# courtois-neuromod/phantom_vlb

Measured on AMD Instinct MI355X. Metric: clips/sec fine-tune VideoLLaMA2-7B+LoRA->2k-voxel head, 1/2/4/8 MI355X, higher is better.
Workload: dtype bf16; 1 GPU; configs[2]: VideoLLaMA2-7B + LoRA r=16 + 2k-voxel head, bf16; clips_per_gpu=3, global_batch=3, seq_len=2048, frames=12, num_target=2048, weights=random-init, comm=none

## Files before the change

include/vlb.h:

```cpp
#ifndef VLB_H
#define VLB_H

#include <stdint.h>

#ifdef __cplusplus
extern "C" {
#endif
#if defined(__GNUC__) || defined(__clang__)
#pragma GCC visibility push(default)
#endif

#define VLB_OK 0
#define VLB_ERR_INVALID (-1)
#define VLB_ERR_LAUNCH (-2)

#define VLB_ABI_VERSION 2

#define VLB_ACT_NONE 0
#define VLB_ACT_QUICK_GELU 1
#define VLB_ACT_GELU 2
#define VLB_ACT_SILU 3
#define VLB_ACT_SWIGLU_PAIR 4
#define VLB_ACT_SWIGLU_BWD 5

int vlb_abi_version(void);
const char* vlb_last_error(void);

int vlb_gemm_bf16(const void* A, int lda, const void* W, int ldw, void* C, int ldc, int M, int N, int K,
                  const void* bias, const void* residual, int ldr, int act, const void* A2, int lda2,
                  const void* W2, int ldw2, int K2, void* stream);

int vlb_gemm_bf16_ws(const void* A, int lda, const void* W, int ldw, void* C, int ldc, int M, int N, int K,
                     const void* bias, const void* residual, int ldr, int act, const void* A2, int lda2,
                     const void* W2, int ldw2, int K2, void* ws, int64_t ws_bytes, void* stream);
int vlb_gemm_swiglu_save(const void* A, int lda, const void* W_il, int ldw, void* H, int ldh, void* GU, int ldgu, int M, int N,
                         int K, const void* A2, int lda2, const void* W2_il, int ldw2, int K2, void* ws, int64_t ws_bytes,
                         void* stream);
int64_t vlb_gemm_workspace_bytes(void);
int vlb_gemm_plan(int M, int N, int K, int K2, int with_workspace);

int vlb_gemm_bf16_masked_pair(const void* A, int lda, const void* W, int ldw, void* C, int ldc, int M, int N, int K,
                              const void* A2, int lda2, const void* W2, int ldw2, float drop_p, uint32_t seed,
                              void* stream);

int vlb_gemm_bf16_masked_pair_ws(const void* A, int lda, const void* W, int ldw, void* C, int ldc, int M, int N, int K,
                                 const void* A2, int lda2, const void* W2, int ldw2, float drop_p, uint32_t seed,
                                 void* ws, int64_t ws_bytes, void* stream);

int vlb_gemm_masked_pair_swiglu_bwd(const void* dY, int lddy, const void* Wt, int ldw, const void* gu, int ldgu, void* dgu,
                                    int lddgu, int M, int ff, int K, const void* U, int ldu, const void* At, int ldat,
                                    float drop_p, uint32_t seed, void* ws, int64_t ws_bytes, void* stream);

int vlb_gemm_kernel_choice(int M, int N, int K, int K2);

int vlb_transpose_bf16(const void* in, void* out, int R, int C, void* stream);

int vlb_attention_fwd(const void* q, int ldq, const void* k, int ldk, const void* v, int ldv, void* out, int ldo,
                      float* lse, const uint8_t* key_mask, int B, int S, int Hq, int Hkv, int D, int causal,
                      float scale, const int* cu_rows, void* stream);

int vlb_attention_bwd(const void* q, int ldq, const void* k, int ldk, const void* v, int ldv, const void* out,
                      int ldo, const void* dout, int lddo, const float* lse, const uint8_t* key_mask, void* dq,
                      int lddq, void* dk, int lddk, void* dv, int lddv, float* delta, float* dq_acc, int B, int S,
                      int Hq, int Hkv, int D, int causal, float scale, const int* cu_rows, int total_rows,
                      void* stream);

int vlb_rmsnorm_fwd(const void* x, const void* w, void* y, int rows, int dim, float eps, void* stream);
int vlb_rmsnorm_bwd(const void* x, const void* w, const void* dy, const void* dx_in, void* dx, int rows, int dim,
                    float eps, void* stream);
int vlb_layernorm_fwd(const void* x, const void* w, const void* b, const void* residual, void* y, int rows, int dim,
                      float eps, int act, void* stream);

int vlb_rope_inplace(void* x, int ld, const float* cos_t, const float* sin_t, int rows, int S, int heads, int D,
                     int sign, const int* pos, void* stream);
int vlb_swiglu_fwd(const void* gu, void* out, int rows, int ff, void* stream);
int vlb_swiglu_bwd(const void* gu, const void* dout, void* dgu, int rows, int ff, void* stream);
int vlb_add_bf16(const void* a, const void* b, void* y, int64_t n, void* stream);

int vlb_patchify(const float* vision, void* patches, int N, int H, int W, int P, int Kpad, void* stream);
int vlb_vit_assemble(const void* patch_emb, const void* cls, const void* pos, void* tokens, int N, int G, int D,
                     void* stream);
int vlb_drop_cls(const void* tokens, void* out, int N, int G, int D, void* stream);

int vlb_dwconv3x3(const void* x, const void* w, void* y, int N, int H, int W, int C, void* stream);
int vlb_se_pool(const void* x, void* pooled, int N, int HW, int C, void* stream);
int vlb_se_scale(const void* x, const void* gate, void* y, int N, int HW, int C, void* stream);
int vlb_im2col3d_k2s2p1(const void* x, void* cols, int B, int T, int H, int W, int C, void* stream);

int vlb_splice_embed(const int64_t* ids, const void* embed_w, const void* video_tokens, void* embeds,
                     uint8_t* key_mask, int* err_flag, int B, int L, int Nv, int D, int64_t video_id, int vocab,
                     const int* cu_rows, int* row_pos, void* stream);
int vlb_weight_mask(const int64_t* padvals, const double* vis_w, const double* lang_w, float* wmask, int B, int F,
                    int Lw, int tokens_per_frame, int S, int round_bf16, void* stream);

int vlb_head_partial_rows(int S);
int64_t vlb_head_ws_floats(int B, int S, int E, int V);
int vlb_head_fwd(const void* hidden, const float* wmask, const void* ln1_w, const void* ln1_b, const void* ln2_w,
                 const void* ln2_b, const void* ridge_w, const void* ridge_b, const float* y, const float* keep_scale,
                 float* ws, float* stats, float* pooled_raw, float* sumw, float* zhat, float* ln2_rstd, void* z,
                 float* pred, float* loss_terms, int B, int S, int E, int V, float eps, float l2_lambda, const int* cu_rows,
                 void* stream);
int vlb_head_bwd(const void* hidden, const float* wmask, const void* ln1_w, const void* ln2_w, const void* ridge_w,
                 const float* y, const float* keep_scale, const float* stats, const float* pooled_raw,
                 const float* sumw, const float* zhat, const float* ln2_rstd, const void* z, const float* pred,
                 float* d_ridge_w, float* d_ridge_b, float* d_ln2_w, float* d_ln2_b, float* d_ln1_w, float* d_ln1_b,
                 float* ws, float* dz_ws, float* dpooled_ws, void* dhidden, int B, int S, int E, int V, float eps,
                 float l2_lambda, float loss_scale, float l2_scale, const int* cu_rows, int total_rows, void* stream);

int vlb_feature_cache_store(const float* pooled_raw, const float* sumw, const int32_t* rows, float* cache_pooled,
                            float* cache_sumw, int B, int E, int n_rows, void* stream);
int vlb_head_fwd_cached(const float* cache_pooled, const float* cache_sumw, const int32_t* rows, const void* ln1_w,
                        const void* ln1_b, const void* ln2_w, const void* ln2_b, const void* ridge_w, const void* ridge_b,
                        const float* y, const float* keep_scale, float* ws, float* pooled_raw, float* sumw, float* zhat,
                        float* ln2_rstd, void* z, float* pred, float* loss_terms, int B, int E, int V, int n_rows, float eps,
                        float l2_lambda, void* stream);
int vlb_head_bwd_cached(const void* ln1_w, const void* ln2_w, const void* ridge_w, const float* y, const float* keep_scale,
                        const float* pooled_raw, const float* sumw, const float* zhat, const float* ln2_rstd, const void* z,
                        const float* pred, float* d_ridge_w, float* d_ridge_b, float* d_ln2_w, float* d_ln2_b, float* d_ln1_w,
                        float* d_ln1_b, float* ws, float* dz_ws, float* dpooled_ws, int B, int E, int V, float eps,
                        float l2_lambda, float loss_scale, float l2_scale, void* stream);

#define VLB_LOSS_MSE 0
#define VLB_LOSS_COSINE 1
#define VLB_LOSS_PEARSON 2
int vlb_head_loss_fwd(const float* pred, const float* y, const float* ws, float* rowstat, float* loss_terms, float* loss_aux,
                      int B, int S, int E, int V, int loss_kind, float l2_lambda, void* stream);
int vlb_head_bwd_loss(const void* hidden, const float* wmask, const void* ln1_w, const void* ln2_w, const void* ridge_w,
                      const float* y, const float* keep_scale, const float* stats, const float* pooled_raw,
                      const float* sumw, const float* zhat, const float* ln2_rstd, const void* z, const float* pred,
                      float* d_ridge_w, float* d_ridge_b, float* d_ln2_w, float* d_ln2_b, float* d_ln1_w, float* d_ln1_b,
                      float* ws, float* dz_ws, float* dpooled_ws, void* dhidden, int B, int S, int E, int V, float eps,
                      float l2_lambda, float loss_scale, float l2_scale, const int* cu_rows, int total_rows, void* stream,
                      int loss_kind, const float* rowstat);
int vlb_head_bwd_cached_loss(const void* ln1_w, const void* ln2_w, const void* ridge_w, const float* y, const float* keep_scale,
                             const float* pooled_raw, const float* sumw, const float* zhat, const float* ln2_rstd,
                             const void* z, const float* pred, float* d_ridge_w, float* d_ridge_b, float* d_ln2_w,
                             float* d_ln2_b, float* d_ln1_w, float* d_ln1_b, float* ws, float* dz_ws, float* dpooled_ws, int B,
                             int E, int V, float eps, float l2_lambda, float loss_scale, float l2_scale, void* stream,
                             int loss_kind, const float* rowstat);

int vlb_head_pool(const void* hidden, const float* wmask, float* ws, float* stats, float* pooled_raw, float* sumw, int B,
                  int S, int E, float eps, const int* cu_rows, void* stream);
int vlb_feature_cache_gather(const float* cache_pooled, const float* cache_sumw, const int32_t* rows, float* pooled_raw,
                             float* sumw, int B, int E, int n_rows, void* stream);
int vlb_head_mix_fwd(const float* p_stack, const void* a, float* alpha, float* pooled_raw, int K, int B, int E,
                     void* stream);
int64_t vlb_head_mix_ws_floats(int K, int B, int E);
int vlb_head_mix_bwd(const float* p_stack, const float* draw, const float* alpha, float* d_a, float* draw_stack, float* ws,
                     int K, int B, int E, void* stream);
int vlb_head_dhidden(const void* hidden, const float* wmask, const float* stats, const float* draw, void* dx, int B, int S,
                     int E, const int* cu_rows, int total_rows, int accumulate, void* stream);

int vlb_lora_down(const void* x, int ldx, const void* A, void* t, int ldt, int M, int K, int R, float scale,
                  float drop_p, const uint32_t* seeds_host, void* stream);
int vlb_lora_merge(const void* W, int ldw, void* Wm, int ldwm, const void* Bt, const void* A, int N, int K, int R, float scale,
                   int row_map, void* stream);
int vlb_lora_dx_masked(const void* u, int ldu, const void* At, int ldat, void* dx, int lddx, int M, int K, int R, float drop_p,
                       const uint32_t* seeds_host, void* stream);
int64_t vlb_wgrad_u_ws_floats(int M, int K);
int vlb_wgrad_skinny_u(const void* G, int ldg, const void* X, int ldx, float* dW, float* ws, int M, int K, float alpha,
                       float beta, const void* Bt, float u_scale, void* u, int ldu, float* u_ws, void* stream);
int vlb_wgrad_skinny_u_multi(const void* G, int ldg, const void* X, int ldx, int M, int nproj, const int* cols, float* const* dW,
                             const void* const* Bt, float* ws, float alpha, float beta, float u_scale, void* u, int ldu,
                             float* u_ws, void* stream);
int vlb_transpose16_scatter(const void* jobs, int n_jobs, void* stream);
int vlb_wgrad_splits(int M);
int vlb_wgrad_skinny(const void* G, int ldg, const void* X, int ldx, float* dW, float* ws, int M, int N, int K,
                     float alpha, float beta, float drop_p, const uint32_t* seeds_host, void* stream);

// ... 77 lines not shown
```

phantom_vlb_amd/_lib.py:

```python
from __future__ import annotations

import ctypes
import os
from ctypes import c_char_p, c_double, c_float, c_int, c_int64, c_void_p

import torch

_HERE = os.path.dirname(os.path.abspath(__file__))
LIB_PATH = os.environ.get("VLB_LIB") or os.path.join(_HERE, "libvlb.so")
IS_PRODUCT_LIB = os.path.abspath(LIB_PATH) == os.path.join(_HERE, "libvlb.so")

P, I, F, L = c_void_p, c_int, c_float, c_int64

SIGNATURES = {
    "vlb_abi_version": [],
    "vlb_last_error": [],
    "vlb_gemm_bf16": [P, I, P, I, P, I, I, I, I, P, P, I, I, P, I, P, I, I, P],
    "vlb_gemm_bf16_ws": [P, I, P, I, P, I, I, I, I, P, P, I, I, P, I, P, I, I, P, L, P],
    "vlb_gemm_swiglu_save": [P, I, P, I, P, I, P, I, I, I, I, P, I, P, I, I, P, L, P],
    "vlb_gemm_workspace_bytes": [],
    "vlb_gemm_plan": [I, I, I, I, I],
    "vlb_gemm_kernel_choice": [I, I, I, I],
    "vlb_transpose_bf16": [P, P, I, I, P],
    "vlb_attention_fwd": [P, I, P, I, P, I, P, I, P, P, I, I, I, I, I, I, F, P, P],
    "vlb_attention_bwd": [P, I, P, I, P, I, P, I, P, I, P, P, P, I, P, I, P, I, P, P, I, I, I, I, I, I, F, P, I, P],
    "vlb_rmsnorm_fwd": [P, P, P, I, I, F, P],
    "vlb_rmsnorm_bwd": [P, P, P, P, P, I, I, F, P],
    "vlb_layernorm_fwd": [P, P, P, P, P, I, I, F, I, P],
    "vlb_rope_inplace": [P, I, P, P, I, I, I, I, I, P, P],
    "vlb_swiglu_fwd": [P, P, I, I, P],
    "vlb_swiglu_bwd": [P, P, P, I, I, P],
    "vlb_add_bf16": [P, P, P, L, P],
    "vlb_patchify": [P, P, I, I, I, I, I, P],
    "vlb_vit_assemble": [P, P, P, P, I, I, I, P],
    "vlb_drop_cls": [P, P, I, I, I, P],
    "vlb_dwconv3x3": [P, P, P, I, I, I, I, P],
    "vlb_se_pool": [P, P, I, I, I, P],
    "vlb_se_scale": [P, P, P, I, I, I, P],
    "vlb_im2col3d_k2s2p1": [P, P, I, I, I, I, I, P],
    "vlb_splice_embed": [P, P, P, P, P, P, I, I, I, I, L, I, P, P, P],
    "vlb_weight_mask": [P, P, P, P, I, I, I, I, I, I, P],
    "vlb_head_partial_rows": [I],
    "vlb_head_ws_floats": [I, I, I, I],
    "vlb_head_fwd": [P] * 19 + [I, I, I, I, F, F, P, P],
    "vlb_head_bwd": [P] * 24 + [I, I, I, I, F, F, F, F, P, I, P],
    "vlb_feature_cache_store": [P] * 5 + [I, I, I, P],
    "vlb_head_fwd_cached": [P] * 19 + [I, I, I, I, F, F, P],
    "vlb_head_bwd_cached": [P] * 20 + [I, I, I, F, F, F, F, P],
    "vlb_head_loss_fwd": [P] * 6 + [I, I, I, I, I, F, P],
    "vlb_head_bwd_loss": [P] * 24 + [I, I, I, I, F, F, F, F, P, I, P, I, P],
    "vlb_head_bwd_cached_loss": [P] * 20 + [I, I, I, F, F, F, F, P, I, P],
    "vlb_head_pool": [P] * 6 + [I, I, I, F, P, P],
    "vlb_feature_cache_gather": [P] * 5 + [I, I, I, P],
    "vlb_head_mix_fwd": [P] * 4 + [I, I, I, P],
    "vlb_head_mix_ws_floats": [I, I, I],
    "vlb_head_mix_bwd": [P] * 6 + [I, I, I, P],
    "vlb_head_dhidden": [P] * 5 + [I, I, I, P, I, I, P],
    "vlb_gemm_bf16_masked_pair": [P, I, P, I, P, I, I, I, I, P, I, P, I, F, ctypes.c_uint32, P],
    "vlb_gemm_masked_pair_swiglu_bwd": [P, I, P, I, P, I, P, I, I, I, I, P, I, P, I, F, ctypes.c_uint32, P, L, P],
    "vlb_gemm_bf16_masked_pair_ws": [P, I, P, I, P, I, I, I, I, P, I, P, I, F, ctypes.c_uint32, P, L, P],
    "vlb_wgrad_u_ws_floats": [I, I],
    "vlb_wgrad_skinny_u": [P, I, P, I, P, P, I, I, F, F, P, F, P, I, P, P],
    "vlb_wgrad_skinny_u_multi": [P, I, P, I, I, I, P, P, P, P, F, F, F, P, I, P, P],
    "vlb_transpose16_scatter": [P, I, P],
    "vlb_wgrad_splits": [I],
    "vlb_wgrad_skinny": [P, I, P, I, P, P, I, I, I, F, F, F, P, P],
    "vlb_lora_down": [P, I, P, P, I, I, I, I, F, F, P, P],
    "vlb_lora_merge": [P, I, P, I, P, P, I, I, I, F, I, P],
    "vlb_lora_dx_masked": [P, I, P, I, P, I, I, I, I, F, P, P],
    "vlb_sumsq_ws_floats": [],
    "vlb_grad_sumsq": [P, L, P, P, P],
    "vlb_adamw_step": [P, P, P, P, P, L, F, F, F, F, F, I, P, F, P],
    "vlb_grad_accum": [P, P, L, I, P, P, P],
    "vlb_grad_accum_bf16": [P, P, L, I, P, P, P],
    "vlb_dropout_keep_scale": [P, L, F, ctypes.c_uint32, P],
    "vlb_transpose_pad": [P, I, P, I, I, I, I, P],
    "vlb_norm_bwd_ws_floats": [I, I],
    "vlb_colsum_ws_floats": [I, I],
    "vlb_rmsnorm_bwd_dw": [P, P, P, P, I, I, F, P],
    "vlb_rmsnorm_bwd_full_ws_floats": [I, I],
    "vlb_rmsnorm_bwd_full": [P, P, P, P, P, P, P, I, I, F, P],
    "vlb_layernorm_bwd": [P, P, P, P, P, P, P, P, P, P, I, I, F, I, P],
    "vlb_act_fwd": [P, P, L, I, P],
    "vlb_act_bwd": [P, P, P, L, I, P],
    "vlb_colsum": [P, I, P, P, I, I, P],
    "vlb_embed_grad": [P, I, P, P, P, I, P, I, P],
    "vlb_grad_sumsq_bf16": [P, L, P, P, P],
    "vlb_adamw_step_g16": [P, P, P, P, P, L, F, F, F, F, F, I, P, F, P],
    "vlb_dwconv3x3_bwd_w_ws_floats": [I, I, I],
    "vlb_dwconv3x3_bwd_w": [P, P, P, P, I, I, I, I, P],
    "vlb_se_bwd_gate": [P, P, P, P, I, I, I, P],
    "vlb_se_bwd_x": [P, P, P, P, I, I, I, P],
    "vlb_col2im3d_k2s2p1": [P, P, I, I, I, I, I, P],
    "vlb_quantize_mxfp8": [P, I, P, I, P, I, I, I, P],
    "vlb_transpose_quantize_mxfp8": [P, I, P, I, P, I, I, I, I, P],
    "vlb_quantize_dual_mxfp8": [P, I, P, I, P, I, P, I, P, I, I, I, I, P],
    "vlb_rmsnorm_fwd_mxfp8": [P, P, P, P, I, P, I, I, I, F, P],
    "vlb_swiglu_fwd_mxfp8": [P, P, P, I, P, I, I, I, P],
    "vlb_gemm_mxfp8": [P, I, P, I, P, I, P, I, P, I, I, I, I, P, I, P],
    "vlb_comm_unique_id": [P],
    "vlb_comm_init": [I, I, P, ctypes.POINTER(c_void_p)],
    "vlb_comm_destroy": [P],
    "vlb_comm_loopback_stage_bytes": [I],
    "vlb_comm_init_loopback": [I, P, L, ctypes.POINTER(c_void_p)],
    "vlb_comm_rank": [P],
    "vlb_comm_world": [P],
    "vlb_allgather_direct": [P, P, P, L, P],
    "vlb_reducescatter_stage_floats": [L, I],
    "vlb_reducescatter_direct": [P, P, P, L, P, P],
    "vlb_reducescatter_direct_bf16": [P, P, P, L, P, P],
    "vlb_reduce_slices": [P, P, L, I, I, P],
    "vlb_profile_marker": [P],
    "vlb_hrf_pool_ws_floats": [I, I],
    "vlb_hrf_pool": [P, I, P, P, P, I, I, I, P],
    "vlb_ridge_ws_floats": [I],
    "vlb_ridge_fwd": [P, P, P, P, P, P, I, I, I, F, P],
    "vlb_allreduce_scalar": [P, P, I, P],
    "vlb_cast_f32_to_bf16": [P, P, L, P],
    "vlb_cast_bf16_to_f32": [P, P, L, P],
}
_RESTYPES = {"vlb_last_error": c_char_p, "vlb_hrf_pool_ws_floats": c_int64, "vlb_ridge_ws_floats": c_int64, "vlb_head_ws_floats": c_int64, "vlb_head_mix_ws_floats": c_int64, "vlb_wgrad_u_ws_floats": c_int64,
# ... 33 lines not shown
```

phantom_vlb_amd/backbone.py:

```python
from __future__ import annotations

import math

import torch

from . import ops
from .geometry import Geometry, VIDEO_TOKEN_ID, decoder_linears

BF16 = torch.bfloat16
V_PRE = "model.vision_tower.vision_tower.vision_model"
M_PRE = "model.mm_projector"


def _bf(t, dev):
    return t.detach().to(device=dev, dtype=BF16).contiguous()


class Weights:

    def __init__(self, g: Geometry, sd: dict, device, keep_transposed: bool = False, gate_up_interleaved: bool | None = None):
        self.g = g
        self.dev = device
        d = device
        w = sd[f"{V_PRE}.embeddings.patch_embedding.weight"].reshape(g.vit_dim, -1)
# ... 89 lines not shown
        sd[f"{V_PRE}.pre_layrnorm.bias"] = zeros(g.vit_dim)
        for i in range(g.vit_layers):
            p = f"{V_PRE}.encoder.layers.{i}"
            for ln in ("layer_norm1", "layer_norm2"):
                sd[f"{p}.{ln}.weight"] = ones(g.vit_dim)
                sd[f"{p}.{ln}.bias"] = zeros(g.vit_dim)
            for n in ("q_proj", "k_proj", "v_proj", "out_proj"):
                sd[f"{p}.self_attn.{n}.weight"] = rn(g.vit_dim, g.vit_dim)
                sd[f"{p}.self_attn.{n}.bias"] = zeros(g.vit_dim)
            sd[f"{p}.mlp.fc1.weight"] = rn(g.vit_ff, g.vit_dim)
            sd[f"{p}.mlp.fc1.bias"] = zeros(g.vit_ff)
            sd[f"{p}.mlp.fc2.weight"] = rn(g.vit_dim, g.vit_ff)
            sd[f"{p}.mlp.fc2.bias"] = zeros(g.vit_dim)
        for st, cin in (("s1", g.vit_dim), ("s2", g.dim)):
            for b in range(g.proj_depth):
                ci = cin if b == 0 else g.dim
                q = f"{M_PRE}.{st}.b{b + 1}"
                rd = int(round(ci * g.proj_se_ratio))
                sd[f"{q}.conv1.conv.weight"] = rn(g.dim, ci, 1, 1, std=1 / math.sqrt(ci))
                sd[f"{q}.conv2.conv.weight"] = rn(g.dim, 1, 3, 3, std=1 / 3)
                sd[f"{q}.se.fc1.weight"] = rn(rd, g.dim, 1, 1, std=1 / math.sqrt(g.dim))
                sd[f"{q}.se.fc1.bias"] = zeros(rd)
                sd[f"{q}.se.fc2.weight"] = rn(g.dim, rd, 1, 1, std=1 / math.sqrt(rd))
                sd[f"{q}.se.fc2.bias"] = zeros(g.dim)
                sd[f"{q}.conv3.conv.weight"] = rn(g.dim, g.dim, 1, 1, std=1 / math.sqrt(g.dim))
                for n in ("conv1", "conv2", "conv3"):
                    sd[f"{q}.{n}.bn.weight"] = ones(g.dim)
                    sd[f"{q}.{n}.bn.bias"] = zeros(g.dim)
                if ci != g.dim:
                    sd[f"{q}.downsample.conv.weight"] = rn(g.dim, ci, 1, 1, std=1 / math.sqrt(ci))
                    sd[f"{q}.downsample.bn.weight"] = ones(g.dim)
                    sd[f"{q}.downsample.bn.bias"] = zeros(g.dim)
        sd[f"{M_PRE}.sampler.0.weight"] = rn(g.dim, g.dim, 2, 2, 2, std=1 / math.sqrt(8 * g.dim))
        sd[f"{M_PRE}.sampler.0.bias"] = zeros(g.dim)
        for n in ("readout.0", "readout.2"):
            sd[f"{M_PRE}.{n}.weight"] = rn(g.dim, g.dim, std=1 / math.sqrt(g.dim))
            sd[f"{M_PRE}.{n}.bias"] = zeros(g.dim)
        sd["model.embed_tokens.weight"] = rn(g.vocab, g.dim)
        for i in range(g.layers):
            p = f"model.layers.{i}"
            for lin in decoder_linears(g):
                sd[f"{p}.{lin.suffix}.weight"] = rn(lin.out, lin.inp)
            sd[f"{p}.input_layernorm.weight"] = ones(g.dim)
            sd[f"{p}.post_attention_layernorm.weight"] = ones(g.dim)
        sd["model.norm.weight"] = ones(g.dim)
        return sd


def destack_decoder_layer(g: Geometry, wqkv, wo, wdown, wgu=None, wgu_il=None) -> dict:
    if wgu is None:
        wgu = wgu_il.view(g.ff // 16, 2, 16, -1).transpose(0, 1).reshape(2 * g.ff, -1)
    stacked = dict(wqkv=wqkv, wo=wo, wgu=wgu, wdown=wdown)
    return {lin.suffix: stacked[lin.stacked][lin.row:lin.row + lin.out] for lin in decoder_linears(g)}


class Backbone:

    def __init__(self, g: Geometry, weights: Weights):
        self.g = g
        self.w = weights
        self.err_flag = torch.zeros(1, dtype=torch.int32, device=weights.dev)

    def vision_tower(self, vision_f32):
        g, w = self.g, self.w
        N = vision_f32.shape[0]
        G, T = g.grid * g.grid, g.grid * g.grid + 1
        hd = g.vit_dim // g.vit_heads
        patches = ops.patchify(vision_f32, g.patch, g.patch_k_padded)
        pe = ops.gemm(patches, w.patch_w)
        x = ops.vit_assemble(pe, w.cls, w.pos, N, G, g.vit_dim)
        x = ops.layernorm(x, *w.pre_ln, g.vit_eps)
        D = g.vit_dim
        for lw in w.vit:
            h = ops.layernorm(x, *lw["ln1"], g.vit_eps)
            qkv = ops.gemm(h, lw["wqkv"], bias=lw["bqkv"])
            a = ops.attention_fwd(qkv[:, :D], qkv[:, D:2 * D], qkv[:, 2 * D:], N, T, g.vit_heads, g.vit_heads, hd,
                                  False, hd ** -0.5)
            x = ops.gemm(a, lw["wo"], bias=lw["bo"], residual=x)
            h = ops.layernorm(x, *lw["ln2"], g.vit_eps)
            h = ops.gemm(h, lw["w1"], bias=lw["b1"], act=ops.ACT_QUICK_GELU)
            x = ops.gemm(h, lw["w2"], bias=lw["b2"], residual=x)
        return ops.drop_cls(x, N, G, D)

    def _bottleneck(self, x, blk, N, H):
        g = self.g
        C = g.dim
        y = ops.gemm(x, blk["conv1"])
        y = ops.layernorm(y, *blk["bn1"], g.proj_eps, act=ops.ACT_SILU)
        y = ops.dwconv3x3(y, blk["dw"], N, H, H, C)
        y = ops.layernorm(y, *blk["bn2"], g.proj_eps, act=ops.ACT_SILU)
        s = ops.se_pool(y, N, H * H, C)
        s = ops.gemm(s, blk["se1"], bias=blk["se1b"], act=ops.ACT_SILU)
        s = ops.gemm(s, blk["se2"], bias=blk["se2b"])
        y = ops.se_scale(y, s, N, H * H, C, out=y)
        y = ops.gemm(y, blk["conv3"])
        sc = x
        if "ds" in blk:
            sc = ops.layernorm(ops.gemm(x, blk["ds"]), *blk["dsbn"], g.proj_eps)
        return ops.layernorm(y, *blk["bn3"], g.proj_eps, residual=sc, act=ops.ACT_SILU)

    def connector(self, feats, B):
        g, w = self.g, self.w
        x = feats
        for blk in w.s1:
            x = self._bottleneck(x, blk, B * g.num_frames, g.grid)
        cols = ops.im2col3d(x, B, g.num_frames, g.grid, g.grid, g.dim)
        x = ops.gemm(cols, w.sampler_w, bias=w.sampler_b, act=ops.ACT_SILU)
        for blk in w.s2:
            x = self._bottleneck(x, blk, B * g.ds_frames, g.ds_grid)
        x = ops.gemm(x, w.ro0[0], bias=w.ro0[1], act=ops.ACT_GELU)
        return ops.gemm(x, w.ro2[0], bias=w.ro2[1])

    def attention(self, qkv, key_mask, B, layout=None, need_lse=False):
        g, w = self.g, self.w
        qd, kd = g.q_dim, g.kv_dim
        ops.rope_(qkv, w.rope_cos, w.rope_sin, B, g.max_len, g.heads + g.kv_heads, g.head_dim,
                  pos=None if layout is None else layout.pos)
        return ops.attention_fwd(qkv[:, :qd], qkv[:, qd:qd + kd], qkv[:, qd + kd:], B, g.max_len, g.heads, g.kv_heads,
                                 g.head_dim, True, g.head_dim ** -0.5, key_mask=key_mask, need_lse=need_lse, layout=layout)

    def attention_bwd(self, qkv, a, d_a, lse, key_mask, B, layout, delta):
        g, w = self.g, self.w
        dqkv = ops.attention_bwd(qkv, g.q_dim, g.kv_dim, a, d_a, lse, key_mask, B, g.max_len, g.heads, g.kv_heads,
                                 g.head_dim, True, g.head_dim ** -0.5, layout=layout, delta=delta)
        ops.rope_(dqkv, w.rope_cos, w.rope_sin, B, g.max_len, g.heads + g.kv_heads, g.head_dim, sign=-1,
                  pos=None if layout is None else layout.pos)
        return dqkv

    def decoder_layer(self, x, lw, key_mask, B, S, save=None, layout=None):
        g = self.g
        assert S == g.max_len, "the decoder runs at the geometry's sequence length (rope tables, attention)"
        h = ops.rmsnorm(x, lw["in_norm"], g.rms_eps)
        qkv = ops.gemm(h, lw["wqkv"])
        a = self.attention(qkv, key_mask, B, layout)
        x = ops.gemm(a, lw["wo"], residual=x)
        h = ops.rmsnorm(x, lw["post_norm"], g.rms_eps)
        if lw.get("wgu_il") is not None:
            h = ops.gemm(h, lw["wgu_il"], act=ops.ACT_SWIGLU_PAIR)
        else:
            h = ops.swiglu(ops.gemm(h, lw["wgu"]))
        return ops.gemm(h, lw["wdown"], residual=x)

    def named_modules(self):
        from .litmodule import _LinearInfo
        g = self.g
        for i in range(g.vit_layers):
            p = f"{V_PRE}.encoder.layers.{i}"
            for n in ("q_proj", "k_proj", "v_proj", "out_proj"):
                yield f"{p}.self_attn.{n}", _LinearInfo(g.vit_dim, g.vit_dim)
            yield f"{p}.mlp.fc1", _LinearInfo(g.vit_ff, g.vit_dim)
            yield f"{p}.mlp.fc2", _LinearInfo(g.vit_dim, g.vit_ff)
        for n in ("readout.0", "readout.2"):
            yield f"{M_PRE}.{n}", _LinearInfo(g.dim, g.dim)
        for i in range(g.layers):
            p = f"model.layers.{i}"
            for lin in decoder_linears(g):
                yield f"{p}.{lin.suffix}", _LinearInfo(lin.out, lin.inp)
        yield "lm_head", _LinearInfo(g.vocab, g.dim)

    def splice(self, ids, video_tokens, layout=None):
        g = self.g
        return ops.splice_embed(ids, self.w.embed, video_tokens, g.vis_tokens, VIDEO_TOKEN_ID, self.err_flag, layout)

    def row_layout(self, ids_host=None, padvals=None):
        g = self.g
        if ids_host is None or ids_host.device.type != "cpu":
            return None
        B, L = ids_host.shape
        S = L - 1 + g.vis_tokens
        nz = ids_host != 0
        last = L - 1 - torch.flip(nz, dims=[1]).to(torch.int8).argmax(dim=1)
        lens = (last + g.vis_tokens).clamp(max=S)
        lens = torch.where(nz.any(dim=1), lens, torch.full_like(lens, S))
        if padvals is not None:
            lens = torch.maximum(lens, S - padvals[:, 0].to(lens.dtype).cpu().clamp(min=0))
        return ops.RowLayout(B, S, lens.tolist(), device=self.w.dev)
# ... 134 lines not shown
```

phantom_vlb_amd/ops.py:

```python
from __future__ import annotations

import torch

from ._lib import check, lib

ACT_NONE, ACT_QUICK_GELU, ACT_GELU, ACT_SILU, ACT_SWIGLU_PAIR = 0, 1, 2, 3, 4
BF16 = torch.bfloat16


def _stream():
    return torch.cuda.current_stream().cuda_stream


def _p(t):
    return None if t is None else t.data_ptr()


def _dev(t):
    if not t.is_cuda:
        raise RuntimeError("phantom_vlb_amd ops need GPU tensors (no CPU fallback)")
    return t


class _GemmProbe:
# ... 280 lines not shown

def rmsnorm_bwd(x, w, dy, eps, dx_in=None, out=None):
    rows, dim = x.shape
    if out is None:
        out = torch.empty_like(x)
    check(lib.vlb_rmsnorm_bwd(_dev(x).data_ptr(), w.data_ptr(), dy.data_ptr(), _p(dx_in), out.data_ptr(), rows, dim, eps,
                              _stream()), "vlb_rmsnorm_bwd")
    return out


def layernorm(x, w, b, eps, residual=None, act=ACT_NONE, out=None):
    rows, dim = x.shape
    if out is None:
        out = torch.empty_like(x)
    check(lib.vlb_layernorm_fwd(_dev(x).data_ptr(), w.data_ptr(), b.data_ptr(), _p(residual), out.data_ptr(), rows, dim,
                                eps, act, _stream()), "vlb_layernorm_fwd")
    return out


def rope_(x, cos, sin, B, S, heads, D, sign=1, pos=None):
    rows = B * S if pos is None else pos.shape[0]
    assert x.shape[0] == rows and cos.shape[0] >= S
    check(lib.vlb_rope_inplace(_dev(x).data_ptr(), x.stride(0), cos.data_ptr(), sin.data_ptr(), rows, S, heads, D, sign,
                               _p(pos), _stream()), "vlb_rope_inplace")
    return x


def swiglu(gu, out=None):
    rows, ff2 = gu.shape
    if out is None:
        out = torch.empty(rows, ff2 // 2, dtype=BF16, device=gu.device)
    check(lib.vlb_swiglu_fwd(_dev(gu).data_ptr(), out.data_ptr(), rows, ff2 // 2, _stream()), "vlb_swiglu_fwd")
    return out


def swiglu_bwd(gu, dout, out=None):
    rows, ff2 = gu.shape
    if out is None:
        out = torch.empty_like(gu)
    check(lib.vlb_swiglu_bwd(_dev(gu).data_ptr(), dout.data_ptr(), out.data_ptr(), rows, ff2 // 2, _stream()), "vlb_swiglu_bwd")
    return out


def add(a, b, out=None):
    if out is None:
        out = torch.empty_like(a)
    check(lib.vlb_add_bf16(_dev(a).data_ptr(), b.data_ptr(), out.data_ptr(), a.numel(), _stream()), "vlb_add_bf16")
    return out


def patchify(vision_f32, P, Kpad):
    N, C, H, W = vision_f32.shape
    assert C == 3 and vision_f32.dtype == torch.float32 and vision_f32.is_contiguous()
    out = torch.empty(N * (H // P) * (W // P), Kpad, dtype=BF16, device=vision_f32.device)
    check(lib.vlb_patchify(_dev(vision_f32).data_ptr(), out.data_ptr(), N, H, W, P, Kpad, _stream()), "vlb_patchify")
    return out


def vit_assemble(patch_emb, cls, pos, N, G, D):
    out = torch.empty(N * (G + 1), D, dtype=BF16, device=patch_emb.device)
    check(lib.vlb_vit_assemble(_dev(patch_emb).data_ptr(), cls.data_ptr(), pos.data_ptr(), out.data_ptr(), N, G, D,
                               _stream()), "vlb_vit_assemble")
    return out


def drop_cls(tokens, N, G, D):
    out = torch.empty(N * G, D, dtype=BF16, device=tokens.device)
    check(lib.vlb_drop_cls(_dev(tokens).data_ptr(), out.data_ptr(), N, G, D, _stream()), "vlb_drop_cls")
    return out


def dwconv3x3(x, w9, N, H, W, C):
    out = torch.empty_like(x)
    check(lib.vlb_dwconv3x3(_dev(x).data_ptr(), w9.data_ptr(), out.data_ptr(), N, H, W, C, _stream()), "vlb_dwconv3x3")
    return out


def se_pool(x, N, HW, C):
    out = torch.empty(N, C, dtype=BF16, device=x.device)
    check(lib.vlb_se_pool(_dev(x).data_ptr(), out.data_ptr(), N, HW, C, _stream()), "vlb_se_pool")
    return out


def se_scale(x, gate, N, HW, C, out=None):
    if out is None:
        out = torch.empty_like(x)
    check(lib.vlb_se_scale(_dev(x).data_ptr(), gate.data_ptr(), out.data_ptr(), N, HW, C, _stream()), "vlb_se_scale")
    return out


def im2col3d(x, B, T, H, W, C):
    T2, H2, W2 = T // 2 + 1, H // 2 + 1, W // 2 + 1
    out = torch.empty(B * T2 * H2 * W2, 8 * C, dtype=BF16, device=x.device)
    check(lib.vlb_im2col3d_k2s2p1(_dev(x).data_ptr(), out.data_ptr(), B, T, H, W, C, _stream()), "vlb_im2col3d_k2s2p1")
    return out


def splice_embed(ids, embed_w, video_tokens, Nv, video_id, err_flag, layout=None):
    B, L = ids.shape
    D = embed_w.shape[1]
    S = L - 1 + Nv
    assert ids.dtype == torch.int64 and ids.is_contiguous()
    packed = layout is not None and layout.packed
    if packed:
        assert layout.B == B and layout.S == S
    rows = layout.rows if packed else B * S
    out = torch.empty(rows, D, dtype=BF16, device=ids.device)
    mask = torch.empty((rows,) if packed else (B, S), dtype=torch.uint8, device=ids.device)
    check(lib.vlb_splice_embed(_dev(ids).data_ptr(), embed_w.data_ptr(), video_tokens.data_ptr(), out.data_ptr(),
                               mask.data_ptr(), err_flag.data_ptr(), B, L, Nv, D, video_id, embed_w.shape[0],
                               _p(layout.cu) if packed else None, _p(layout.pos) if packed else None,
                               _stream()), "vlb_splice_embed")
    return out, mask


def weight_mask(padvals, vis_w, lang_w, tokens_per_frame, S, round_bf16=True):
    B, F = vis_w.shape
    assert padvals.dtype == torch.int64 and vis_w.dtype == torch.float64 and lang_w.dtype == torch.float64
    out = torch.empty(B, S, dtype=torch.float32, device=padvals.device)
    check(lib.vlb_weight_mask(_dev(padvals).contiguous().data_ptr(), vis_w.contiguous().data_ptr(),
                              lang_w.contiguous().data_ptr(), out.data_ptr(), B, F, lang_w.shape[1], tokens_per_frame, S,
                              1 if round_bf16 else 0, _stream()), "vlb_weight_mask")
    return out


def dropout_keep_scale(B, E, p, seed, device):
    out = torch.empty(B, E, dtype=torch.float32, device=device)
    check(lib.vlb_dropout_keep_scale(_dev(out).data_ptr(), out.numel(), float(p), int(seed) & 0xFFFFFFFF, _stream()),
          "vlb_dropout_keep_scale")
    return out


def profile_marker():
    check(lib.vlb_profile_marker(_stream()), "vlb_profile_marker")


def cast_bf16(x_f32):
    out = torch.empty(x_f32.shape, dtype=BF16, device=x_f32.device)
    check(lib.vlb_cast_f32_to_bf16(_dev(x_f32).data_ptr(), out.data_ptr(), x_f32.numel(), _stream()), "vlb_cast_f32_to_bf16")
    return out


_ws_cache = {}


def _ws(n_floats, device, tag="norm"):
    key = (device.index, tag)
    buf = _ws_cache.get(key)
    if buf is None or buf.numel() < n_floats:
        buf = _ws_cache[key] = torch.empty(int(n_floats), dtype=torch.float32, device=device)
    return buf


def transpose_pad(x, out, rows_pad):
    R, C = x.shape
    assert out.shape[0] >= C and out.stride(1) == 1 and x.stride(1) == 1 and rows_pad % 8 == 0 and out.shape[1] >= rows_pad
    check(lib.vlb_transpose_pad(_dev(x).data_ptr(), x.stride(0), out.data_ptr(), out.stride(0), R, C, rows_pad, _stream()),
          "vlb_transpose_pad")
    return out


def rmsnorm_bwd_dw(x, dy, eps, out):
    rows, dim = x.shape
    ws = _ws(lib.vlb_norm_bwd_ws_floats(rows, dim), x.device)
    check(lib.vlb_rmsnorm_bwd_dw(_dev(x).data_ptr(), dy.data_ptr(), out.data_ptr(), ws.data_ptr(), rows, dim, eps, _stream()),
          "vlb_rmsnorm_bwd_dw")
# ... 138 lines not shown
```

Baseline: 15.26 clips/s.

## Fuse SE layernorm with pooling and add skinny MFMA GEMM for SE FCs

In the connector bottleneck blocks, the second layernorm+SiLU now also accumulates per-block column sums, and a small finalize kernel turns them into the SE pooled vector. This removes the separate se_pool pass that re-read the full activation. The two SE fully-connected layers, which have at most 64 rows, now use a new split-K MFMA skinny GEMM in place of the general GEMM path. The cost is an extra fp32 partials buffer and two new kernels. The new vision.hip file must also be built into the library.

New measurement: 15.25 clips/s (median of 2 runs). About the same (-0.0%).

```diff
diff --git a/include/vlb.h b/include/vlb.h
--- a/include/vlb.h
+++ b/include/vlb.h
@@ -85,6 +85,12 @@
 int vlb_dwconv3x3(const void* x, const void* w, void* y, int N, int H, int W, int C, void* stream);
 int vlb_se_pool(const void* x, void* pooled, int N, int HW, int C, void* stream);
 int vlb_se_scale(const void* x, const void* gate, void* y, int N, int HW, int C, void* stream);
+int vlb_gemm_skinny_bf16(const void* x, int ldx, const void* W, int ldw, const void* bias, int act, void* y, int ldy, int M, int N,
+                         int K, void* stream);
+int vlb_layernorm_pool_parts(int N, int HW);
+int vlb_layernorm_pool_fwd(const void* x, const void* w, const void* b, void* y, float* partials, int N, int HW, int dim, float eps,
+                           int act, void* stream);
+int vlb_se_pool_finalize(const float* partials, void* pooled, int N, int parts, int HW, int C, void* stream);
 int vlb_im2col3d_k2s2p1(const void* x, void* cols, int B, int T, int H, int W, int C, void* stream);
 
 int vlb_splice_embed(const int64_t* ids, const void* embed_w, const void* video_tokens, void* embeds,
diff --git a/phantom_vlb_amd/_lib.py b/phantom_vlb_amd/_lib.py
--- a/phantom_vlb_amd/_lib.py
+++ b/phantom_vlb_amd/_lib.py
@@ -37,6 +37,10 @@
     "vlb_dwconv3x3": [P, P, P, I, I, I, I, P],
     "vlb_se_pool": [P, P, I, I, I, P],
     "vlb_se_scale": [P, P, P, I, I, I, P],
+    "vlb_gemm_skinny_bf16": [P, I, P, I, P, I, P, I, I, I, I, P],
+    "vlb_layernorm_pool_parts": [I, I],
+    "vlb_layernorm_pool_fwd": [P, P, P, P, P, I, I, I, F, I, P],
+    "vlb_se_pool_finalize": [P, P, I, I, I, I, P],
     "vlb_im2col3d_k2s2p1": [P, P, I, I, I, I, I, P],
     "vlb_splice_embed": [P, P, P, P, P, P, I, I, I, I, L, I, P, P, P],
     "vlb_weight_mask": [P, P, P, P, I, I, I, I, I, I, P],
diff --git a/phantom_vlb_amd/backbone.py b/phantom_vlb_amd/backbone.py
--- a/phantom_vlb_amd/backbone.py
+++ b/phantom_vlb_amd/backbone.py
@@ -195,16 +195,21 @@
             x = ops.gemm(h, lw["w2"], bias=lw["b2"], residual=x)
         return ops.drop_cls(x, N, G, D)
 
+    @staticmethod
+    def _se_fc(s, w, b, act):
+        if s.shape[0] <= 64 and w.shape[0] % 16 == 0 and w.shape[1] % 64 == 0:
+            return ops.gemm_skinny(s, w, bias=b, act=act)
+        return ops.gemm(s, w, bias=b, act=act)
+
     def _bottleneck(self, x, blk, N, H):
         g = self.g
         C = g.dim
         y = ops.gemm(x, blk["conv1"])
         y = ops.layernorm(y, *blk["bn1"], g.proj_eps, act=ops.ACT_SILU)
         y = ops.dwconv3x3(y, blk["dw"], N, H, H, C)
-        y = ops.layernorm(y, *blk["bn2"], g.proj_eps, act=ops.ACT_SILU)
-        s = ops.se_pool(y, N, H * H, C)
-        s = ops.gemm(s, blk["se1"], bias=blk["se1b"], act=ops.ACT_SILU)
-        s = ops.gemm(s, blk["se2"], bias=blk["se2b"])
+        y, s = ops.layernorm_pool(y, *blk["bn2"], g.proj_eps, N, H * H, act=ops.ACT_SILU)
+        s = self._se_fc(s, blk["se1"], blk["se1b"], ops.ACT_SILU)
+        s = self._se_fc(s, blk["se2"], blk["se2b"], ops.ACT_NONE)
         y = ops.se_scale(y, s, N, H * H, C, out=y)
         y = ops.gemm(y, blk["conv3"])
         sc = x
diff --git a/phantom_vlb_amd/csrc/vision.hip b/phantom_vlb_amd/csrc/vision.hip
--- /dev/null
+++ b/phantom_vlb_amd/csrc/vision.hip
@@ -0,0 +1,234 @@
+#include "common.hpp"
+
+namespace {
+
+__device__ __forceinline__ float act_f(float x, int act) {
+  switch (act) {
+    case VLB_ACT_QUICK_GELU: return quick_gelu_f(x);
+    case VLB_ACT_GELU: return gelu_erf_f(x);
+    case VLB_ACT_SILU: return silu_f(x);
+    default: return x;
+  }
+}
+
+constexpr int SK_WAVES = 16;
+constexpr int SK_KC = 64;
+
+template <int MT>
+__global__ __launch_bounds__(1024) void gemm_skinny_kernel(const bf16* __restrict__ x, int ldx, const bf16* __restrict__ W, int ldw,
+                                                           const bf16* __restrict__ bias, bf16* __restrict__ y, int ldy, int M, int K,
+                                                           int act) {
+  extern __shared__ __attribute__((aligned(16))) char sk_lds[];
+  f32x4* red = reinterpret_cast<f32x4*>(sk_lds);
+  const int lane = threadIdx.x & 63, wave = threadIdx.x >> 6;
+  const int fr = lane & 15, fq = lane >> 4;
+  const int n0 = blockIdx.x * 16;
+  const bf16* wp = W + (int64_t)(n0 + fr) * ldw + fq * 8;
+  const bf16* xp[MT];
+#pragma unroll
+  for (int t = 0; t < MT; ++t) xp[t] = x + (int64_t)min(t * 16 + fr, M - 1) * ldx + fq * 8;
+  f32x4 acc[MT];
+#pragma unroll
+  for (int t = 0; t < MT; ++t) acc[t] = f32x4{0.f, 0.f, 0.f, 0.f};
+  for (int k = wave * SK_KC; k < K; k += SK_WAVES * SK_KC) {
+    const bf16x8 w0 = *reinterpret_cast<const bf16x8*>(wp + k);
+    const bf16x8 w1 = *reinterpret_cast<const bf16x8*>(wp + k + 32);
+    bf16x8 a0[MT], a1[MT];
+#pragma unroll
+    for (int t = 0; t < MT; ++t) {
+      a0[t] = *reinterpret_cast<const bf16x8*>(xp[t] + k);
+      a1[t] = *reinterpret_cast<const bf16x8*>(xp[t] + k + 32);
+    }
+#pragma unroll
+    for (int t = 0; t < MT; ++t) {
+      acc[t] = __builtin_amdgcn_mfma_f32_16x16x32_bf16(w0, a0[t], acc[t], 0, 0, 0);
+      acc[t] = __builtin_amdgcn_mfma_f32_16x16x32_bf16(w1, a1[t], acc[t], 0, 0, 0);
+    }
+  }
+#pragma unroll
+  for (int t = 0; t < MT; ++t) red[(wave * MT + t) * 64 + lane] = acc[t];
+  __syncthreads();
+  if (wave >= MT) return;
+  f32x4 s = red[wave * 64 + lane];
+  for (int w = 1; w < SK_WAVES; ++w) {
+    const f32x4 p = red[(w * MT + wave) * 64 + lane];
+#pragma unroll
+    for (int e = 0; e < 4; ++e) s[e] += p[e];
+  }
+  const int m = wave * 16 + fr;
+  if (m >= M) return;
+  const int n = n0 + fq * 4;
+  bf16x4 o;
+#pragma unroll
+  for (int e = 0; e < 4; ++e) {
+    float v = s[e];
+    if (bias) v += (float)bias[n + e];
+    o[e] = (bf16)act_f(v, act);
+  }
+  *reinterpret_cast<bf16x4*>(y + (int64_t)m * ldy + n) = o;
+}
+
+template <int NI>
+__global__ __launch_bounds__(256, 3) void layernorm_pool_kernel(const bf16* __restrict__ x, const bf16* __restrict__ w,
+                                                             const bf16* __restrict__ b, bf16* __restrict__ y,
+                                                             float* __restrict__ part, int HW, int rpb, int dim, float eps, int act) {
+  __shared__ __attribute__((aligned(16))) float red[3][NI * 512];
+  bf16* sw = reinterpret_cast<bf16*>(&red[0][0]);
+  bf16* sb = sw + NI * 512;
+  const int lane = threadIdx.x & 63, wave = threadIdx.x >> 6;
+  const int64_t n = blockIdx.y;
+  for (int c = threadIdx.x * 8; c < dim; c += 256 * 8) {
+    *reinterpret_cast<bf16x8*>(sw + c) = *reinterpret_cast<const bf16x8*>(w + c);
+    *reinterpret_cast<bf16x8*>(sb + c) = *reinterpret_cast<const bf16x8*>(b + c);
+  }
+  __syncthreads();
+  const int r0 = blockIdx.x * rpb, r1 = min(r0 + rpb, HW);
+  float cs[NI][8];
+#pragma unroll
+  for (int k = 0; k < NI; ++k)
+#pragma unroll
+    for (int i = 0; i < 8; ++i) cs[k][i] = 0.f;
+  for (int r = r0 + wave; r < r1; r += 4) {
+    const int64_t row = n * HW + r;
+    const bf16* xr = x + row * dim;
+    bf16x8 xb[NI];
+#pragma unroll
+    for (int k = 0; k < NI; ++k) {
+      const int c = lane * 8 + k * 512;
+      xb[k] = c < dim ? *reinterpret_cast<const bf16x8*>(xr + c) : bf16x8{};
+    }
+    float s = 0.f;
+#pragma unroll
+    for (int k = 0; k < NI; ++k)
+#pragma unroll
+      for (int i = 0; i < 8; ++i) s += (float)xb[k][i];
+    const float mean = wave_sum(s) / dim;
+    float ss = 0.f;
+#pragma unroll
+    for (int k = 0; k < NI; ++k) {
+      if (lane * 8 + k * 512 < dim) {
+#pragma unroll
+        for (int i = 0; i < 8; ++i) { const float d = (float)xb[k][i] - mean; ss += d * d; }
+      }
+    }
+    const float rstd = rsqrtf(wave_sum(ss) / dim + eps);
+    bf16* yr = y + row * dim;
+#pragma unroll
+    for (int k = 0; k < NI; ++k) {
+      const int c = lane * 8 + k * 512;
+      if (c < dim) {
+        const bf16x8 g = *reinterpret_cast<const bf16x8*>(sw + c), bb = *reinterpret_cast<const bf16x8*>(sb + c);
+        float v[8];
+#pragma unroll
+        for (int i = 0; i < 8; ++i) v[i] = ((float)xb[k][i] - mean) * rstd * (float)g[i] + (float)bb[i];
+        if (act != VLB_ACT_NONE) {
+#pragma unroll
+          for (int i = 0; i < 8; ++i) v[i] = act_f(v[i], act);
+        }
+        bf16x8 o;
+#pragma unroll
+        for (int i = 0; i < 8; ++i) { o[i] = (bf16)v[i]; cs[k][i] += (float)o[i]; }
+        *reinterpret_cast<bf16x8*>(yr + c) = o;
+      }
+    }
+  }
+  __syncthreads();
+  if (wave > 0) {
+#pragma unroll
+    for (int k = 0; k < NI; ++k) {
+      float* d = &red[wave - 1][lane * 8 + k * 512];
+      *reinterpret_cast<f32x4*>(d) = f32x4{cs[k][0], cs[k][1], cs[k][2], cs[k][3]};
+      *reinterpret_cast<f32x4*>(d + 4) = f32x4{cs[k][4], cs[k][5], cs[k][6], cs[k][7]};
+    }
+  }
+  __syncthreads();
+  if (wave > 0) return;
+  float* pr = part + (n * gridDim.x + blockIdx.x) * dim;
+#pragma unroll
+  for (int k = 0; k < NI; ++k) {
+    const int c = lane * 8 + k * 512;
+    if (c < dim) {
+      float o[8];
+#pragma unroll
+      for (int i = 0; i < 8; ++i) o[i] = ((cs[k][i] + red[0][c + i]) + red[1][c + i]) + red[2][c + i];
+      *reinterpret_cast<f32x4*>(pr + c) = f32x4{o[0], o[1], o[2], o[3]};
+      *reinterpret_cast<f32x4*>(pr + c + 4) = f32x4{o[4], o[5], o[6], o[7]};
+    }
+  }
+}
+
+__global__ __launch_bounds__(256) void se_pool_finalize_kernel(const float* __restrict__ part, bf16* __restrict__ pooled, int parts,
+                                                               int HW, int C) {
+  const int c = (blockIdx.x * 256 + threadIdx.x) * 4;
+  if (c >= C) return;
+  const int64_t n = blockIdx.y;
+  const float* p = part + n * parts * C + c;
+  f32x4 s = *reinterpret_cast<const f32x4*>(p);
+  for (int i = 1; i < parts; ++i) {
+    const f32x4 t = *reinterpret_cast<const f32x4*>(p + (int64_t)i * C);
+#pragma unroll
+    for (int e = 0; e < 4; ++e) s[e] += t[e];
+  }
+  bf16x4 o;
+#pragma unroll
+  for (int e = 0; e < 4; ++e) o[e] = (bf16)(s[e] / HW);
+  *reinterpret_cast<bf16x4*>(pooled + n * C + c) = o;
+}
+
+int pool_rows_per_block(int N, int HW) {
+  int rpb = 32;
+  while (rpb > 8 && (int64_t)N * ((HW + rpb - 1) / rpb) < 384) rpb >>= 1;
+  return rpb;
+}
+
+}
+
+extern "C" int vlb_gemm_skinny_bf16(const void* x, int ldx, const void* W, int ldw, const void* bias, int act, void* y, int ldy,
+                                    int M, int N, int K, void* stream) {
+  VLB_REQUIRE(M > 0 && M <= 64 && N > 0 && N % 16 == 0 && K > 0 && K % 64 == 0, "gemm_skinny: need 0 < M <= 64, N %% 16 == 0, K %% 64 == 0 (M=%d N=%d K=%d)",
+              M, N, K);
+  VLB_REQUIRE(ldx >= K && ldw >= K && ldy >= N && ldx % 8 == 0 && ldw % 8 == 0 && ldy % 4 == 0 && ((uintptr_t)x % 16) == 0 &&
+                  ((uintptr_t)W % 16) == 0 && ((uintptr_t)y % 8) == 0,
+              "gemm_skinny: rows of x and W must be 16-byte aligned, rows of y 8-byte aligned");
+  VLB_REQUIRE(act == VLB_ACT_NONE || act == VLB_ACT_QUICK_GELU || act == VLB_ACT_GELU || act == VLB_ACT_SILU, "gemm_skinny: act=%d", act);
+  const int mt = (M + 15) / 16;
+#define VLB_SK_LAUNCH(MT)                                                                                                        \
+  hipLaunchKernelGGL(gemm_skinny_kernel<MT>, dim3(N / 16), dim3(SK_WAVES * 64), SK_WAVES * MT * 1024, as_stream(stream), (const bf16*)x, \
+                     ldx, (const bf16*)W, ldw, (const bf16*)bias, (bf16*)y, ldy, M, K, act)
+  if (mt == 1) VLB_SK_LAUNCH(1);
+  else if (mt == 2) VLB_SK_LAUNCH(2);
+  else if (mt == 3) VLB_SK_LAUNCH(3);
+  else VLB_SK_LAUNCH(4);
+#undef VLB_SK_LAUNCH
+  VLB_LAUNCH_CHECK();
+  return VLB_OK;
+}
+
+extern "C" int vlb_layernorm_pool_parts(int N, int HW) {
+  if (N <= 0 || HW <= 0) return 0;
+  const int rpb = pool_rows_per_block(N, HW);
+  return (HW + rpb - 1) / rpb;
+}
+
+extern "C" int vlb_layernorm_pool_fwd(const void* x, const void* w, const void* b, void* y, float* partials, int N, int HW, int dim,
+                                      float eps, int act, void* stream) {
+  VLB_REQUIRE(N > 0 && HW > 0 && dim > 0 && dim % 8 == 0 && dim <= 4096, "layernorm_pool_fwd: dim=%d must be a multiple of 8, at most 4096", dim);
+  VLB_REQUIRE(partials && ((uintptr_t)partials % 16) == 0, "layernorm_pool_fwd: partials must be 16-byte aligned");
+  const int rpb = pool_rows_per_block(N, HW);
+#define VLB_LP_ARGS dim3((HW + rpb - 1) / rpb, N), dim3(256), 0, as_stream(stream), (const bf16*)x, (const bf16*)w, (const bf16*)b, \
+                    (bf16*)y, partials, HW, rpb, dim, eps, act
+  if (dim <= 512) hipLaunchKernelGGL(layernorm_pool_kernel<1>, VLB_LP_ARGS);
+  else if (dim <= 1024) hipLaunchKernelGGL(layernorm_pool_kernel<2>, VLB_LP_ARGS);
+  else hipLaunchKernelGGL(layernorm_pool_kernel<8>, VLB_LP_ARGS);
+#undef VLB_LP_ARGS
+  VLB_LAUNCH_CHECK();
+  return VLB_OK;
+}
+
+extern "C" int vlb_se_pool_finalize(const float* partials, void* pooled, int N, int parts, int HW, int C, void* stream) {
+  VLB_REQUIRE(N > 0 && parts > 0 && HW > 0 && C > 0 && C % 8 == 0, "se_pool_finalize: bad shape");
+  hipLaunchKernelGGL(se_pool_finalize_kernel, dim3((C / 4 + 255) / 256, N), dim3(256), 0, as_stream(stream), partials, (bf16*)pooled,
+                     parts, HW, C);
+  VLB_LAUNCH_CHECK();
+  return VLB_OK;
+}
diff --git a/phantom_vlb_amd/ops.py b/phantom_vlb_amd/ops.py
--- a/phantom_vlb_amd/ops.py
+++ b/phantom_vlb_amd/ops.py
@@ -386,6 +386,31 @@
     return out
 
 
+def layernorm_pool(x, w, b, eps, N, HW, act=ACT_NONE, out=None):
+    rows, dim = x.shape
+    assert rows == N * HW and x.is_contiguous()
+    if out is None:
+        out = torch.empty_like(x)
+    parts = lib.vlb_layernorm_pool_parts(N, HW)
+    part = torch.empty(N, parts, dim, dtype=torch.float32, device=x.device)
+    pooled = torch.empty(N, dim, dtype=BF16, device=x.device)
+    check(lib.vlb_layernorm_pool_fwd(_dev(x).data_ptr(), w.data_ptr(), b.data_ptr(), out.data_ptr(), part.data_ptr(), N, HW, dim,
+                                     eps, act, _stream()), "vlb_layernorm_pool_fwd")
+    check(lib.vlb_se_pool_finalize(part.data_ptr(), pooled.data_ptr(), N, parts, HW, dim, _stream()), "vlb_se_pool_finalize")
+    return out, pooled
+
+
+def gemm_skinny(x, w, bias=None, act=ACT_NONE, out=None):
+    M, K = x.shape
+    N = w.shape[0]
+    assert w.shape[1] == K and x.stride(1) == 1 and w.stride(1) == 1
+    if out is None:
+        out = torch.empty(M, N, dtype=BF16, device=x.device)
+    check(lib.vlb_gemm_skinny_bf16(_dev(x).data_ptr(), x.stride(0), w.data_ptr(), w.stride(0), _p(bias), act, out.data_ptr(),
+                                   out.stride(0), M, N, K, _stream()), "vlb_gemm_skinny_bf16")
+    return out
+
+
 def se_scale(x, gate, N, HW, C, out=None):
     if out is None:
         out = torch.empty_like(x)
```
